# Paleogenomics/IBDGem

Hardware: AMD Instinct MI355X
Metric: SNP-sites/sec in --LD mode, chr1, 2504-indiv panel (higher is better)
Workload: dtype f64

## Files before the change

ibdgem_amd/csrc/ibdg_api.cpp:

```cpp
#include "../../include/ibdgem_hip.h"
#include "ibdg_ctx.h"
#include "ibdg_kernels.h"
#include "ibdg_states.h"

static_assert(sizeof(ibdg_segment) == 56, "ibdg_segment has no padding");

#include <hip/hip_runtime.h>

#include <cerrno>
#include <unistd.h>
#include <cfloat>
#include <cmath>
#include <cstdarg>
#include <cstdio>
#include <cstdlib>
#include <cstring>
#include <algorithm>
#include <atomic>
#include <chrono>
#include <mutex>
#include <string>
#include <thread>
#include <vector>

// ... 1333 lines not shown
}

int relayout_when_paid(ibdg_ctx *c, size_t T)
{
    if (!(c->tab.pop_lut_ok && c->lay.pop_sites_ok && !c->lay.compact && c->opt.compact == 0 && c->opt.variant != 1 &&
          c->opt.variant != 3 && c->lay.pop_dense_enough))
        return 0;
    const bool to_mfma = c->opt.mfma_targets && c->lay.tab_in_lds && T >= (size_t)c->opt.mfma_min;
    c->lay.relayout_credit += to_mfma ? (uint64_t)((T + IBDG_TG - 1) / IBDG_TG) * 20u : (uint64_t)T * (c->opt.mx_counts ? 12u : 16u);
    if (c->lay.relayout_credit >= (uint64_t)std::max<long>(1, c->opt.compact_targets)) {
        if (quiesce(c)) return 1;
        Built b = build_segments(c, true);
        if (b == Built::not_applicable)
            b = build_segments(c, false);
        return b == Built::failed;
    }
    return 0;
}

struct RunPlan {
    size_t T = 0, lanes = 0;
    bool ld = false, use_pop = false;
    int variant = 0, count_unit = 0;
    bool recount = false, rows_on_main = false, dispatch_events = false, rt_build = false;
    size_t MT = 0, n_gg = 0, T_g = 0, gg_batch = 0, T_cnt = 0, n_grp = 0, T_one = 0;
    bool mfma_wg_sum = false;
    size_t ph_group = 0, part_bytes = 0;
    int mx_counts = 0;
    long rho_shift = 0;
    bool ibd1 = false, ibd0_pass = false, fin_in_next = false, end_in_dispatch = false;
    bool side_fast = false;
    unsigned row_blocks = 0;
};

int plan_run(ibdg_ctx *c, size_t T, size_t lanes, int ld_mode, bool row_table, RunPlan &P)
{
    P.T = T; P.lanes = lanes; P.ld = ld_mode != 0;
    P.rt_build = row_table && !c->rt.fresh(*c);
    if (ld_mode) {
        const bool can = c->tab.pop_lut_ok && c->lay.pop_sites_ok && (c->lay.compact ? c->lay.t32c.p : c->pan.t32.p);
        if (c->opt.variant == 2 && !can)
            return fail(c, "[::] ERROR in ibdg_run: ld_variant 2 (exponent counting) is not applicable here "
                           "(clamped P(D|G) table, epsilon outside (0,1), max_cov > 50 or rows out of order)");
        P.use_pop = can && c->opt.variant != 1 && c->opt.variant != 3 && (c->opt.variant == 2 || c->lay.pop_dense_enough);
    }
    P.variant = ld_mode ? (P.use_pop ? 2 : (c->opt.variant == 3 ? 3 : 1)) : 0;
    P.recount = c->opt.count_in_run || !c->pan.counts_valid;
    P.rows_on_main = !ld_mode && !P.recount;
    P.dispatch_events = P.use_pop && c->opt.dispatch_events && c->sites.n_win > 0;
    if (P.use_pop) {
        P.MT = (size_t)ibdg::ld_popcount_mt_width();
        const bool mt_fits = ibdg::ld_popcount_lds_bytes(c->lay.max_seg, c->lay.wpg, c->lay.ct_max + 1, c->lay.tab_in_lds, c->lay.seg_ring,
                                                         1) <= 150 * 1024;
// ... 8 lines not shown
        }
        P.T_cnt = T - P.T_g;
        P.n_grp = (c->opt.multi_target && mt_fits && P.T_cnt >= P.MT) ? P.T_cnt / P.MT : 0;
        P.T_one = P.T_cnt - P.n_grp * P.MT;
        const size_t mem_cap = std::max<size_t>((size_t)1 << 30, c->dev_mem_bytes / 16);
        const size_t fit = std::min(c->lay.n_segs ? mem_cap / ((size_t)c->lay.n_segs * 1024) : P.n_gg, mem_cap / P.ph_group);
        P.gg_batch = std::min({std::max<size_t>(fit, 1), (size_t)std::max<long>(1, c->opt.mfma_batch), P.n_gg});
        const double log2_rho = std::log2(c->tab.eps / (1 - c->tab.eps)), log2_sigma = std::log2(0.5 / (1 - c->tab.eps));
        const bool shift8 = (double)(c->lay.ct_max + 1) * std::max(std::fabs(log2_rho + 8.0), std::fabs(log2_sigma)) <= 1000.0;
        P.rho_shift = shift8 ? 8 : std::lround(-log2_rho);
        const double per_read = std::max(std::fabs(log2_rho + (double)P.rho_shift), std::fabs(log2_sigma));
        P.mx_counts = c->opt.mx_counts && P.rho_shift >= 0 && P.rho_shift <= 40 &&
                      (!c->lay.tab_in_lds || (double)(c->lay.ct_max + 1) * per_read <= 1000.0) &&
                      ibdg::ld_popcount_lds_bytes(c->lay.max_seg, c->lay.wpg, c->lay.ct_max + 1, c->lay.tab_in_lds, c->lay.seg_ring, 2) <= 150 * 1024;
        P.part_bytes = T * (size_t)c->sites.n_win * c->pan.n_chunks * 16;
        const bool p2_stale = !c->p2.fresh(*c, P.mx_counts);
        if (P.T_one && P.mx_counts && c->lay.tab_in_lds && c->opt.ibd0_after > 0) {
            if (!c->ibd0.fresh(*c))
                c->ibd0.made(*c);
            c->ibd0.ibd0_runs += P.T_one;
            P.ibd1 = !p2_stale || (P.n_gg > 0) || c->ibd0.ibd0_runs >= (uint64_t)c->opt.ibd0_after;
        }
        P.ibd0_pass = p2_stale && (P.n_gg > 0 || P.ibd1);
        P.fin_in_next = c->opt.fin_next && c->opt.async && P.T_one > 0 && P.T_one == P.T_cnt && P.n_gg == 0;
        P.end_in_dispatch = c->opt.end_in_dispatch && P.fin_in_next && !P.dispatch_events && P.T_one == T && !c->opt.log_windows;
        P.count_unit = P.T_one ? (P.mx_counts ? (P.ibd1 ? 3 : 2) : 1) : 0;
        P.side_fast = P.n_gg > 0;
    }
    if (ld_mode && !P.recount && !P.side_fast && c->opt.site_blocks > 0)
        P.row_blocks = std::max<unsigned>(1u, (unsigned)((size_t)c->n_cu * c->opt.site_blocks / T));
    return 0;
}

int start_run(ibdg_ctx *c, const RunPlan &P, EvSet &E, bool flushed)
{
    E.recount = P.recount; E.ld = P.ld; E.rows_on_main = P.rows_on_main; E.has_kernel_times = P.dispatch_events;
    const bool chained = c->tl.chain_ok && c->opt.async;
    if (P.dispatch_events) {
        E.start = E.start_own;
        if (chained)
            HIP_TRY(c, hipStreamWaitEvent(c->stream2, c->tl.evs[c->tl.ev_head].ld_end, 0));
        return 0;
    }
    if (chained && !flushed) {
        E.start = c->tl.evs[c->tl.ev_head].ld_end;
    } else {
        HIP_TRY(c, hipEventRecord(E.start_own, c->stream));
        E.start = E.start_own;
    }
// ... 98 lines not shown
    return 0;
}

int launch_mt_groups(ibdg_ctx *c, const RunPlan &P, const ibdg::PopArgs &pa, ibdg::KernelEvents &first,
                     ibdg::KernelEvents dominant)
{
    if (ring_settle(c)) return 1;
    ibdg::PopArgs pm = pa;
    pm.mx_counts = 0;
    pm.rec_ready = (const uint32_t *)c->twords_mt.p; pm.wc_ready = (const uint32_t *)c->wtarget_mt.p;
    ibdg::launch_win_target_mt(pm, (unsigned)P.n_grp, c->stream, first);
    first = ibdg::KernelEvents();
    if (ibdg::launch_ld_popcount_mt(pm, (unsigned)P.n_grp, c->stream, P.T_one ? ibdg::KernelEvents() : dominant))
        return fail(c, "[::] ERROR in ibdg_run: the multi-target --LD kernel could not be launched");
    return 0;
}

int launch_singles(ibdg_ctx *c, const RunPlan &P, ibdg::PopArgs pa, ibdg::KernelEvents first, ibdg::KernelEvents dominant,
                   bool same_inputs, EvSet &E)
{
    Ring &R = c->ring;
    pa.t_base = (uint32_t)(P.T_g + P.n_grp * P.MT);
    pa.ibd1 = P.ibd1 ? 1u : 0u;
    const ibdg_ctx::Images::Key key = c->img.key_for(*c, pa.t_base, (uint32_t)P.T_one, P.mx_counts, (int)P.ibd1, R.cur);
    const bool wt_cached = same_inputs && c->img.fresh(key) && !P.dispatch_events;
    const bool wt_ahead = R.unsettled && !P.dispatch_events;
    const hipStream_t is = wt_ahead ? c->stream3 : c->stream;
    if (!wt_ahead && ring_settle(c)) return 1;
    if (wt_ahead && R.s3_gen != c->sites_gen) {
        HIP_TRY(c, hipEventRecord(R.ev_s3sync, c->stream));
        HIP_TRY(c, hipStreamWaitEvent(c->stream3, R.ev_s3sync, 0));
        R.s3_gen = c->sites_gen;
    }
    if (P.ibd1) {
        if (!c->fb.fresh(*c)) {
            if (ensure(c, c->fb.fragb, (size_t)c->lay.n_segs * 72)) return 1;
            if (!c->fb.ev_fb)
                HIP_TRY(c, hipEventCreateWithFlags(&c->fb.ev_fb, hipEventDisableTiming));
            ibdg::launch_frag_base(pa, (uint32_t *)c->fb.fragb.p, is);
            HIP_TRY(c, hipEventRecord(c->fb.ev_fb, is));
            HIP_TRY(c, hipStreamWaitEvent(wt_ahead ? c->stream : c->stream3, c->fb.ev_fb, 0));
            c->fb.made(*c);
        }
        pa.frag_base = (const uint32_t *)c->fb.fragb.p;
    }
    if (!wt_cached)
// ... 197 lines not shown
    const size_t lanes = (size_t)c->pan.n_groups * c->pan.cpw * 64;
    const bool want_ll = c->opt.site_results != 0;
    const bool row_table = want_ll && ld_mode;
    if (ensure(c, c->targets, Ring::SLOTS * T * 4) || (want_ll && ensure(c, c->site_ll, (row_table ? 1 : T) * c->sites.n_sites * 24)) ||
        (row_table && ensure(c, c->rt.row_tab, c->sites.n_sites * 32)) || ensure(c, c->win_ll, T * (size_t)c->sites.n_win * 24) ||
        (c->opt.log_windows && ensure(c, c->wlog.win_log2, T * (size_t)c->sites.n_win * 24)))
        return 1;
    const bool same_bg = c->bg.prev_pu == pu_id && c->bg.prev_has_bg == (bg_count ? 1 : 0) && c->bg.prev_lanes == lanes &&
                         (!bg_count || (c->bg.prev_bg.size() == c->pan.n_ids &&
                                        std::equal(bg_count, bg_count + c->pan.n_ids, c->bg.prev_bg.begin()))) &&
                         c->bg.base_w.p;
    const bool same_inputs = same_bg && c->prev_targets.size() == T && std::equal(targets, targets + T, c->prev_targets.begin()) &&
                             c->weight.p;
    if (!same_bg && set_background(c, bg_count, pu_id, lanes)) return 1;
    if (ring_settle(c) || (!same_inputs && ring_prepare(c, targets, T, lanes))) return 1;
    if (ld_mode && relayout_when_paid(c, T)) return 1;
    RunPlan P;
    if (plan_run(c, T, lanes, ld_mode, row_table, P)) return 1;
    const bool ld_log = c->opt.log_windows && ld_mode && c->sites.n_win > 0;
    if (ld_log && ld_log_refused(c))
        return fail(c, "[::] ERROR in ibdg_run: log_windows cannot give the --LD columns here: %s", ld_log_refused(c));
    c->last_variant = P.variant;
    c->last_count_unit = P.count_unit;
    const bool flush = c->fin.pending && (!same_bg || c->fin.sites_gen != c->sites_gen || !P.use_pop || P.ibd0_pass ||
                                          !P.fin_in_next || c->fin.count != (unsigned)P.T_cnt || c->fin.args.t_base != (uint32_t)P.T_g);
    if (flush && flush_finalize(c)) return 1;
    const int ev_slot = (c->tl.ev_head + 1) % ibdg_ctx::Timeline::EV_RING;
    EvSet &E = c->tl.evs[ev_slot];
    if (start_run(c, P, E, flush)) return 1;

    const ibdg::RowsArgs sa = rows_args(c, ld_mode, row_table);
    if (ld_log && launch_log_windows(c, P)) return 1;
    if (P.use_pop ? launch_pop(c, P, E, same_inputs) : ld_mode && launch_strict(c, P, targets, bg_count, pu_id)) return 1;
    if (ring_settle(c)) return 1;
    if (P.rows_on_main) {
        if (join_streams(c)) return 1;
        unsigned blocks = 0;
        if (c->opt.rows_blocks > 0)
            blocks = std::max<unsigned>(1u, (unsigned)((size_t)c->n_cu * c->opt.rows_blocks / T));
        ibdg::launch_rows_windows(sa, (unsigned)T, c->stream, blocks);
        if (c->opt.log_windows)
            ibdg::launch_win_log_rows(sa, (unsigned)T, (double *)c->wlog.win_log2.p, c->stream);
    }
    if (!P.dispatch_events && !P.end_in_dispatch)
        HIP_TRY(c, hipEventRecord(E.ld_end, c->stream));
    if (!P.rows_on_main && queue_stream2(c, P, sa, E)) return 1;
// ... 400 lines not shown
    if (back + 1 >= (unsigned)ibdg_ctx::Timeline::EV_RING || (long)back >= c->tl.runs_done)
        return fail(c, "[::] ERROR in ibdg_run_kernel_ms: no timing kept for the run %u calls back", back);
    const EvSet &E = c->tl.evs[(c->tl.ev_head + ibdg_ctx::Timeline::EV_RING - (int)back) % ibdg_ctx::Timeline::EV_RING];
    if (!E.has_kernel_times)
        return fail(c, "[::] ERROR in ibdg_run_kernel_ms: that run did not use the exponent-counting --LD kernel");
    if (quiesce(c)) return 1;
    HIP_TRY(c, hipEventElapsedTime(ms, E.k_start, E.k_stop));
    return 0;
}

int ibdg_last_run_ms(ibdg_ctx *c, float out[5])
{
    if (!c || !out) return 1;
    if (c->tl.runs_done == 0) {
        for (int i = 0; i < 5; ++i) out[i] = 0.f;
        return 0;
    }
    return ibdg_run_ms(c, 0, out);
}

int ibdg_last_ld_variant(const ibdg_ctx *c) { return c ? c->last_variant : 0; }

int ibdg_last_count_unit(const ibdg_ctx *c) { return c ? c->last_count_unit : 0; }

int ibdg_ld_layout(const ibdg_ctx *c)
{
    if (!c || !c->sites.sites_valid || !c->lay.pop_sites_ok)
        return 0;
    return c->lay.compact ? 2 : 1;
}

int ibdg_set_option(ibdg_ctx *c, const char *name, long value)
{
    if (!c || !name) return 1;
    for (const OptionRow &o : OPTION_TABLE) {
        if (strcmp(name, o.name))
            continue;
        const bool in_set = o.kind == OptionRow::SET && value >= 0 && value < 63 && ((o.lo >> value) & 1);
        if ((o.kind == OptionRow::RANGE && (value < o.lo || value > o.hi)) || (o.kind == OptionRow::SET && !in_set)) {
            if (o.text)
                return fail(c, "[::] ERROR in ibdg_set_option: %s must be %s", o.name, o.text);
            return fail(c, "[::] ERROR in ibdg_set_option: %s must be %ld..%ld", o.name, o.lo, o.hi);
        }
        if (o.effect == OptionRow::JOIN_STREAMS && join_streams(c)) return 1;
        if (o.effect == OptionRow::FIX_WPG) c->opt.wpg_fixed = true;
        c->opt.*o.member = o.kind == OptionRow::BOOL ? value != 0 : o.kind == OptionRow::CLAMP ? std::min(std::max(value, o.lo), o.hi) : value;
// ... 44 lines not shown
```

ibdgem_amd/csrc/ibdg_ctx.h:

```cpp
#pragma once
#include "ibdg_kernels.h"

#include <hip/hip_runtime.h>

#include <climits>
#include <cstddef>
#include <cstdint>
#include <initializer_list>
#include <string>
#include <vector>

struct DevBuf {
    void *p = nullptr;
    size_t cap = 0;
    uint64_t allocs = 0;
    void release()
    {
        if (p)
            (void)hipFree(p);
        p = nullptr;
        cap = 0;
    }
};

// ... 28 lines not shown
        long cpw = 0;
        long waves = 8;
        long variant = 0;
        std::vector<uint32_t> bg_order;
        long wpg = 16;
        bool wpg_fixed = false;
        long multi_target = 1;
        long mfma_targets = 1;
        long mfma_plain_tau = 1;
        long mfma_min = 4;
        long mfma_wg_sum = 1;
        long mfma_batch = 36;
        long guided = 4;
        long ring = 2;
        long recbytes = 12 * 1024;
        long site_blocks = 2;
        long recount_blocks = 4;
        long compact = 0;
        long ibd0_after = 8;
        long prep_ahead = 1;
        long end_in_dispatch = 1;
        long fin_next = 1;
        long sum_dpp = 1;
        long mx_counts = 1;
        long reserve_compact = 1;
        long compact_align = 1;
        long compact_density = 4;
        long compact_targets = 256;
        long site_results = 1;
        long staged_upload = 1;
        long log_windows = 0;
        long stage_workers = Staging::WORKERS;
    } opt;

    struct Tables {
        double eps = 0.02;
        unsigned max_cov = 20;
        std::vector<double> lut_h;
        DevBuf lut;
        bool pop_lut_ok = false;
        std::vector<unsigned long> nck_h;
        DevBuf nck_dev;
        std::vector<ibdg::PowEntry> p1_h, p2_h, p3_h;
        std::vector<ibdg::WinRaw> pb_h;
        DevBuf pow1, pow2, pow3, powb;
        size_t tab_dev = 0;
// ... 167 lines not shown
        bool fresh(Product k, const int64_t want[3]) const
        { return have[k] && P[k][0] == want[0] && P[k][1] == want[1] && P[k][2] == want[2]; }
        void made(Product k, const int64_t made_for[3])
        { have[k] = true; P[k][0] = made_for[0]; P[k][1] = made_for[1]; P[k][2] = made_for[2]; }
        bool records_fresh() const { return recs_ok; }
        void records_made() { recs_ok = true; }
        void records_drop() { recs_ok = false; }
        void drop() { have[PATH] = have[POST] = recs_ok = false; }
        void free_bufs() { release_all({&path, &score, &count, &post, &pout, &ptab, &spos, &sout, &soff, &recs}); }
    } ls;

    struct PendingFin {
        bool pending = false;
        ibdg::PopFinalArgs args;
        unsigned count = 0;
        uint64_t sites_gen = 0;
        int half = 0;
    } fin;

    DevBuf wtarget_mt, twords_mt, partial, aimg, wc_slot, partial_h, vals, order;

    int last_variant = 0;
    int last_count_unit = 0;
    std::vector<uint32_t> prev_targets;
    struct Ring {
        static constexpr int SLOTS = 4;
        static constexpr int NREF_SLOTS = 2 * SLOTS;
        static constexpr size_t AHEAD_MAX_T = 64;
        static constexpr int STAGE_SLOTS = 4;
        uint32_t *stage[STAGE_SLOTS] = {};
        size_t stage_cap = 0;
        hipEvent_t stage_ev[STAGE_SLOTS] = {};
        int stage_next = 0;
        int cur = 0;
        int nref = 0;
        hipEvent_t main_read[SLOTS] = {}, s2_read[SLOTS] = {};
        bool main_pending[SLOTS] = {}, s2_pending[SLOTS] = {};
        hipEvent_t ready = nullptr;
        bool unsettled = false;
        hipEvent_t ev_s3sync = nullptr;
        uint64_t s3_gen = 0;
    } ring;

    DevBuf targets, weight, nrefpanel, af, site_ll, win_ll;
    DevBuf llr_seg, llr_part, llr_out;
    size_t n_targets = 0;
// ... 30 lines not shown
using Opt = ibdg_ctx::Options;
const OptionRow OPTION_TABLE[] = {
    {"count_in_run", &Opt::count_in_run, OptionRow::BOOL},
    {"multi_target", &Opt::multi_target, OptionRow::BOOL},
    {"mfma_targets", &Opt::mfma_targets, OptionRow::BOOL},
    {"mfma_plain_tau", &Opt::mfma_plain_tau, OptionRow::BOOL},
    {"mfma_min", &Opt::mfma_min, OptionRow::RANGE, 1, IBDG_TG},
    {"guided_runs", &Opt::guided, OptionRow::ANY},
    {"compact_align", &Opt::compact_align, OptionRow::SET, opt_set({1, 2, 4, 8, 16, 32}), 0, "1, 2, 4, 8, 16 or 32"},
    {"mfma_wg_sum", &Opt::mfma_wg_sum, OptionRow::BOOL},
    {"mfma_batch_groups", &Opt::mfma_batch, OptionRow::CLAMP, 1, 64},
    {"ibd0_after", &Opt::ibd0_after, OptionRow::CLAMP, 0, LONG_MAX},
    {"end_in_dispatch", &Opt::end_in_dispatch, OptionRow::BOOL},
    {"prep_ahead", &Opt::prep_ahead, OptionRow::BOOL},
    {"dispatch_events", &Opt::dispatch_events, OptionRow::BOOL},
    {"async", &Opt::async, OptionRow::BOOL},
    {"dev_inputs_ready", &Opt::dev_inputs_ready, OptionRow::BOOL},
    {"staged_upload", &Opt::staged_upload, OptionRow::BOOL},
    {"stage_workers", &Opt::stage_workers, OptionRow::RANGE, 1, ibdg_ctx::Staging::WORKERS},
    {"compact_tiles", &Opt::compact, OptionRow::RANGE, -1, 1, "-1 (never), 0 (auto) or 1 (always)"},
    {"finalize_in_next", &Opt::fin_next, OptionRow::RANGE, 0, 1, "0 or 1", OptionRow::JOIN_STREAMS},
    {"sum_dpp", &Opt::sum_dpp, OptionRow::RANGE, 0, 1, "0 or 1"},
    {"mx_counts", &Opt::mx_counts, OptionRow::RANGE, 0, 1, "0 or 1"},
    {"reserve_compact", &Opt::reserve_compact, OptionRow::RANGE, 0, 1, "0 or 1"},
    {"compact_density", &Opt::compact_density, OptionRow::RANGE, 1, 1000000},
    {"compact_targets", &Opt::compact_targets, OptionRow::RANGE, 1, 65536},
    {"site_results", &Opt::site_results, OptionRow::RANGE, 0, 1, "0 or 1"},
    {"log_windows", &Opt::log_windows, OptionRow::RANGE, 0, 1, "0 or 1"},
    {"rows_blocks_per_cu", &Opt::rows_blocks, OptionRow::RANGE, 0, 128},
    {"site_blocks_per_cu", &Opt::site_blocks, OptionRow::RANGE, 0, 128},
    {"recount_blocks_per_cu", &Opt::recount_blocks, OptionRow::RANGE, 0, 128},
    {"chunks_per_wave", &Opt::cpw, OptionRow::RANGE, 0, 5},
    {"waves_per_block", &Opt::waves, OptionRow::RANGE, 1, 8},
    {"ld_variant", &Opt::variant, OptionRow::RANGE, 0, 3, "0 (auto), 1 (strict), 2 (exponent counting) or 3 (reference order)"},
    {"ring_slots", &Opt::ring, OptionRow::SET, opt_set({2, 3, 4, 8}), 0, "2, 3, 4 or 8"},
    {"record_lds_bytes", &Opt::recbytes, OptionRow::RANGE, 1024, 96 * 1024},
    {"windows_per_wave", &Opt::wpg, OptionRow::RANGE, 1, 65536, nullptr, OptionRow::FIX_WPG},
};
```

ibdgem_amd/csrc/ibdg_kernels.h:

```cpp
#pragma once
#include <hip/hip_runtime_api.h>
#include <hip/hip_vector_types.h>
#include <stddef.h>
#include <stdint.h>

struct ibdg_segment;

namespace ibdg {

struct RowsArgs {
    const uint64_t *panel;
    uint32_t stride;
    uint32_t n_ids;
    const uint2 *rec_all;
    size_t n_sites;
    const double *lut;
    const uint32_t *alt_count;
    const double *pow_tab;
    const double *fo;
    const uint32_t *targets;
    const uint4 *t32;
    uint32_t n_pairs;
    const uint32_t *cov_site;
    const uint2 *rec_cov;
// ... 72 lines not shown
    const uint32_t *run_begin;
    uint32_t n_runs;
    uint32_t n_cgroups;
    uint32_t waves_per_group;
    const uint32_t *wc_ready;
    const PowEntry *pow_1me;
    const PowEntry *pow_eps;
    const uint32_t *targets;
    uint32_t t_base;
    const double *weight;
    uint32_t lanes;
    double *partial;
    uint32_t ring_slots;
    uint32_t tab_len;
    uint32_t tab_in_lds;
    uint32_t rho_shift = 0;
    const double *fin_prev = nullptr;
    const int *n_refpanel = nullptr;
    double *win_ll = nullptr;
    uint32_t sum_dpp = 0;
    uint32_t mx_counts = 0;
    double *p2_out = nullptr;
    uint32_t ibd1 = 0;
    const double *fin_p2c = nullptr, *fin_p2w = nullptr;
    const uint32_t *fin_targets = nullptr;
    const uint32_t *frag_base = nullptr;
};

struct KernelEvents {
    hipEvent_t start = nullptr, stop = nullptr;
};

struct PopFinalArgs {
    const WinConst *wconst;
    const double *partial;
    uint32_t n_win, n_chunks;
    const int *n_refpanel;
    double *win_ll;
    uint32_t t_base = 0;
    uint32_t halves = 0;
    uint32_t p_t0 = 0;
    const double *p2c = nullptr, *p2w = nullptr;
    const uint32_t *targets = nullptr;
    uint32_t lanes = 0;
};

// ... 183 lines not shown
```

ibdgem_amd/csrc/ibdg_ld_popcount.hip:

```cpp
#include "ibdg_kernels.h"
#include "ibdg_ld_dev.h"
#include "ibdg_ld_layout.h"

#include <hip/hip_runtime.h>
#include <hip/hip_ext.h>

#include <type_traits>

#ifndef IBDG_TILE_AUX
#define IBDG_TILE_AUX 2
#endif

namespace ibdg {

typedef int mx_v8i __attribute__((ext_vector_type(8)));
typedef float mx_v4f __attribute__((ext_vector_type(4)));
typedef uint32_t mx_u4 __attribute__((ext_vector_type(4)));
typedef uint32_t mx_u2 __attribute__((ext_vector_type(2)));


__device__ __forceinline__ mx_v8i bits_to_fp4(uint32_t x)
{
    mx_v8i b = {0, 0, 0, 0, 0, 0, 0, 0};
    b[0] = (int)(x & 0x11111111u);
// ... 53 lines not shown
    v = swz_add<2>(v);
    v = swz_add<4>(v);
    v = swz_add<8>(v);
    v = swz_add<16>(v);
    return v;
}

__device__ __forceinline__ double wave_sum2_dpp(double a, double b, uint32_t scr_w, uint32_t scr_r)
{
    uint4 r;
    asm volatile("ds_write_b64 %1, %2\n\t"
                 "ds_write_b64 %1, %3 offset:512\n\t"
                 "ds_read_b128 %0, %4\n\t"
                 "s_waitcnt lgkmcnt(0)"
                 : "=&v"(r)
                 : "v"(scr_w), "v"(a), "v"(b), "v"(scr_r)
                 : "memory");
    double v = __hiloint2double((int)r.y, (int)r.x) + __hiloint2double((int)r.w, (int)r.z);
    v = dpp_add<0xB1, 0xf>(v);
    v = dpp_add<0x4E, 0xf>(v);
    v = dpp_add<0x141, 0xf>(v);
    v = dpp_add<0x140, 0xf>(v);
    v = dpp_add<0x142, 0xa>(v);
    return v;
}



__device__ __forceinline__ void lds_fetch(uint4 &h0, uint4 &h1, uint2 &x, uint32_t rec_addr, uint32_t x_addr)
{
    asm volatile("ds_read_b128 %0, %3\n\t"
                 "ds_read_b128 %1, %3 offset:16\n\t"
                 "ds_read_b64 %2, %4\n\t"
                 "s_waitcnt lgkmcnt(0)"
                 : "=&v"(h0), "=&v"(h1), "=&v"(x)
                 : "v"(rec_addr), "v"(x_addr)
                 : "memory");
}

#define IBDG_PAIR_SET(tmp, a, b, cnt) \
    "v_and_b32 %[" #tmp "], %[" #a "], %[" #b "]\n\ts_nop 0\n\tv_bcnt_u32_b32 %[" #cnt "], %[" #tmp "], 0\n\t"
#define IBDG_PAIR_ADD(tmp, a, b, cnt) \
    "v_and_b32 %[" #tmp "], %[" #a "], %[" #b "]\n\ts_nop 0\n\tv_bcnt_u32_b32 %[" #cnt "], %[" #tmp "], %[" #cnt "]\n\t"
#define IBDG_COV_PLANE_TEXT(P, k) \
    P(u0, x0, cov##k, c0##k) P(u1, x1, cov##k, c1##k) P(t, hom, cov##k, ch##k) \
    P(t, u0, at0, g00##k) P(t, u1, at0, g01##k) P(t, u0, at1, g10##k) P(t, u1, at1, g11##k)
// ... 634 lines not shown
            window_end_entries<false>(r, a, t, w, wgt, k0, k1, u, m32);
    }
    ring.drain();
}

__device__ __forceinline__ double ibd1_window_value(const Run &r, const PopArgs &a, const MxCounts &m, uint32_t w, double wgt)
{
    uint4 k0, k1;
    read_window_constants(k0, k1, r, w);
    const int eK = (int)k0.x;
    const uint32_t kc0 = k0.z, kc1 = k0.w, kb0 = k1.x, kb1 = k1.y;
    uint32_t ad[8];
    ad[0] = mad24<8>(__float_as_uint(m.acc0[2]), kb0);   ad[1] = mad24<8>(__float_as_uint(m.acc0[0]), kc0);
    ad[2] = mad24<8>(__float_as_uint(m.acc1[2]), kb0);   ad[3] = mad24<8>(__float_as_uint(m.acc1[0]), kc0);
    ad[4] = mad24<8>(__float_as_uint(m.acc0[3]), kb1);   ad[5] = mad24<8>(__float_as_uint(m.acc0[1]), kc1);
    ad[6] = mad24<8>(__float_as_uint(m.acc1[3]), kb1);   ad[7] = mad24<8>(__float_as_uint(m.acc1[1]), kc1);
    uint2 pq[8];
    lds_read_pow8_b64(pq, ad);
    double val[4];
    ld_products_plain<4>(pq, ad, eK, r.tab1, a.rho_shift, val);
    return wgt * (((val[0] + val[1]) + val[2]) + val[3]);
}

template <class Ring>
__device__ __forceinline__ void run_ibd1_form(Ring &ring, const Run &r, const PopArgs &a, unsigned t)
{
    const double wgt = a.weight[(size_t)(a.t_base + t) * a.lanes + r.c * 64 + r.lane];
    ring.wait_first();
    MxCounts m = {{0.f, 0.f, 0.f, 0.f}, {0.f, 0.f, 0.f, 0.f}, {0, 0, 0, 0}, {0, 0}};
    mx_v4f bias4 = {12582912.f, 12582912.f, 12582912.f, 12582912.f};
    asm volatile("" : "+v"(bias4));
    SegCursor cur = {0, r.rec_addr + 24 * (r.lane & 3), r.x_off0, 0};
    uint32_t w = r.w0;
    while (cur.s < r.nseg) {
        uint32_t flags = segment_x1<true>(ring, cur, r, m, bias4);
        while (!(flags & (1u << 15)))
            flags = segment_x1<false>(ring, cur, r, m, bias4);
        const double tot = wave_sum_lane63_only(ibd1_window_value(r, a, m, w, wgt));
        if (r.lane == 63)
            partial_of(a, r, t, w)[1] = tot;
        ++w;
    }
    ring.drain();
}

__device__ __forceinline__ bool fused_finalize(uint32_t &bx, unsigned t, const WinConst *__restrict__ wconst, const PopArgs &a)
{
    if (!a.fin_prev)
        return false;
    const uint32_t n_fin = (a.n_win + a.waves_per_group - 1) / a.waves_per_group;
    if (bx >= n_fin) {
        bx -= n_fin;
        return false;
    }
    const unsigned wave = __builtin_amdgcn_readfirstlane(threadIdx.x >> 6), lane = threadIdx.x & 63;
    const uint32_t w = bx * a.waves_per_group + wave;
    if (w < a.n_win) {
        const unsigned tt = a.t_base + t;
        double t0 = 0.0, t1 = 0.0;
        chunk_partial_sums(reinterpret_cast<const double2 *>(a.fin_prev) + ((size_t)tt * a.n_win + w) * a.n_chunks, a.n_chunks, lane,
                           t0, t1);
        finalize_window(t0, t1, a.fin_p2c, a.fin_p2w, a.fin_targets, a.lanes, a.n_chunks, a.n_win, w, tt, lane, wconst,
                        a.n_refpanel, a.win_ll, "fused finalize");
    }
    return true;
}

template <int NS, bool TAB_LDS, bool MX, bool IBD1 = false>
__global__ __launch_bounds__(512) void k_ld_popcount(const uint4 *__restrict__ t32,
                                                     const Seg *__restrict__ segs,
                                                     const uint32_t *__restrict__ rec_ready,
                                                     const WinConst *__restrict__ wconst,
                                                     const uint32_t *__restrict__ wc_ready,
                                                     const uint4 *__restrict__ pow_1me,
                                                     const uint4 *__restrict__ pow_eps,
                                                     const uint32_t *__restrict__ run_begin,
                                                     PopArgs a)
{
    static_assert(!IBD1 || (MX && TAB_LDS), "the IBD1 form exists with the counts on the matrix cores and the tables in LDS");
    extern __shared__ __attribute__((aligned(16))) char smem[];
    const unsigned t = blockIdx.z;
    uint32_t bx = blockIdx.x;
    if (fused_finalize(bx, t, wconst, a))
        return;
    const RunSpan sp = run_span(bx, run_begin, wconst, a);
    if (sp.nseg == 0)
        return;
    TileRing<NS, MX> ring;
    const Run r = run_prologue<MX ? IBDG_RECX_WORDS : IBDG_REC_WORDS, IBDG_WC_WORDS, TAB_LDS, MX && TAB_LDS ? 8 : 16, !IBD1>(
        sp, ring, smem, t, t32, segs, rec_ready, wc_ready, pow_1me, pow_eps, a);
    if (!r.has_chunk)
        return;
    if constexpr (IBD1)
        run_ibd1_form(ring, r, a, t);
    else if constexpr (MX)
        run_matrix_form<TAB_LDS>(ring, r, a, t);
    else
        run_vector_form<TAB_LDS>(ring, r, a, t);
}


template <int NS, bool TAB_LDS>
__global__ __launch_bounds__(512) void k_ld_popcount_mt(const uint4 *__restrict__ t32,
                                                        const Seg *__restrict__ segs,
                                                        const uint32_t *__restrict__ rec_ready,
                                                        const WinConst *__restrict__ wconst,
                                                        const uint32_t *__restrict__ wc_ready,
                                                        const uint4 *__restrict__ pow_1me,
                                                        const uint4 *__restrict__ pow_eps,
                                                        const uint32_t *__restrict__ run_begin,
                                                        PopArgs a)
{
    constexpr int TB = IBDG_MT;
    extern __shared__ __attribute__((aligned(16))) char smem[];
    const unsigned g = blockIdx.z;
    const RunSpan sp = run_span(blockIdx.x, run_begin, wconst, a);
    if (sp.nseg == 0)
// ... 71 lines not shown
    if (w >= a.n_win)
        return;
    const unsigned lane = threadIdx.x & 63;
    const unsigned t = blockIdx.y + a.t_base;
    double t0 = 0.0, t1 = 0.0;
    if (a.halves) {
        const double2 *p = reinterpret_cast<const double2 *>(a.partial) + ((size_t)(t - a.p_t0) * a.n_win + w) * a.n_chunks * 2;
        for (uint32_t c = lane; c < a.n_chunks; c += 64) {
            const double2 v = p[2 * c], u = p[2 * c + 1];
            t0 += v.x + u.x;
            t1 += v.y + u.y;
        }
    } else {
        chunk_partial_sums(reinterpret_cast<const double2 *>(a.partial) + ((size_t)(t - a.p_t0) * a.n_win + w) * a.n_chunks,
                           a.n_chunks, lane, t0, t1);
    }
    finalize_window(t0, t1, a.p2c, a.p2w, a.targets, a.lanes, a.n_chunks, a.n_win, w, t, lane, a.wconst, a.n_refpanel, a.win_ll,
                    "k_ld_finalize");
}

size_t ld_popcount_lds_bytes(uint32_t max_seg, uint32_t win_per_group, uint32_t tab_len, int tab_in_lds,
                             int ring_slots, int multi_target)
{
    const bool mt = multi_target == 1, mx = multi_target == 2 || multi_target == 3;
    return ld_lds_layout(max_seg, win_per_group, tab_len, mt ? IBDG_RECM_WORDS : mx ? IBDG_RECX_WORDS : IBDG_REC_WORDS,
                         mt ? IBDG_WCM_WORDS : IBDG_WC_WORDS, tab_in_lds ? (mx ? 8 : 16) : 0,
                         ring_slots, 8, multi_target != 3)
        .bytes;
}

template <class F>
static int with_ring_slots(uint32_t ring_slots, F &&launch)
{
    switch (ring_slots) {
    case 2:
        return launch(std::integral_constant<int, 2>());
    case 3:
        return launch(std::integral_constant<int, 3>());
    case 4:
        return launch(std::integral_constant<int, 4>());
    default:
        return launch(std::integral_constant<int, 8>());
    }
}

using CountKernel = void (*)(const uint4 *, const Seg *, const uint32_t *, const WinConst *, const uint32_t *, const uint4 *,
                             const uint4 *, const uint32_t *, PopArgs);
static int launch_counting(CountKernel kern, size_t lds, const PopArgs &a, dim3 grid, hipStream_t st, KernelEvents ev)
{
    if (hipFuncSetAttribute(reinterpret_cast<const void *>(kern), hipFuncAttributeMaxDynamicSharedMemorySize,
                            (int)lds) != hipSuccess)
        return 1;
    hipExtLaunchKernelGGL(kern, grid, dim3(64 * a.waves_per_group), (uint32_t)lds, st, ev.start, ev.stop, 0,
                          (const uint4 *)a.t32, a.segs, a.rec_ready, a.wconst, a.wc_ready, (const uint4 *)a.pow_1me,
                          (const uint4 *)a.pow_eps, a.run_begin, a);
    return 0;
}

template <int NS, bool TAB, bool MX, bool IBD1 = false>
static int launch_pop(const PopArgs &a, dim3 grid, hipStream_t st, KernelEvents ev)
{
    return launch_counting(k_ld_popcount<NS, TAB, MX, IBD1>,
                           ld_popcount_lds_bytes(a.max_seg, a.win_per_group, a.tab_len, TAB, NS, IBD1 ? 3 : MX ? 2 : 0), a, grid,
                           st, ev);
}

int launch_ld_popcount(const PopArgs &a, unsigned n_targets, int planes, hipStream_t st, KernelEvents ev)
{
    if (a.n_win == 0)
        return 0;
    if (planes < 1 || planes > 8)
        return 1;
    dim3 grid(a.n_runs * a.n_cgroups + (a.fin_prev ? (a.n_win + a.waves_per_group - 1) / a.waves_per_group : 0), 1, n_targets);
    if (a.ibd1 && (!a.mx_counts || !a.tab_in_lds || a.p2_out))
        return 1;
    return with_ring_slots(a.ring_slots, [&](auto ns) {
        constexpr int NS = decltype(ns)::value;
        if (a.ibd1)
            return launch_pop<NS, true, true, true>(a, grid, st, ev);
        if (a.mx_counts)
            return a.tab_in_lds ? launch_pop<NS, true, true>(a, grid, st, ev) : launch_pop<NS, false, true>(a, grid, st, ev);
        return a.tab_in_lds ? launch_pop<NS, true, false>(a, grid, st, ev) : launch_pop<NS, false, false>(a, grid, st, ev);
    });
}

int launch_ld_popcount_mt(const PopArgs &a, unsigned n_groups, hipStream_t st, KernelEvents ev)
{
    if (a.n_win == 0 || n_groups == 0)
        return 0;
    dim3 grid(a.n_runs * a.n_cgroups, 1, n_groups);
    return with_ring_slots(a.ring_slots, [&](auto ns) {
        constexpr int NS = decltype(ns)::value;
        const size_t lds = ld_popcount_lds_bytes(a.max_seg, a.win_per_group, a.tab_len, a.tab_in_lds != 0, NS, 1);
        return launch_counting(a.tab_in_lds ? k_ld_popcount_mt<NS, true> : k_ld_popcount_mt<NS, false>, lds, a, grid, st, ev);
    });
}

void launch_ld_finalize(const PopFinalArgs &a, unsigned n_targets, hipStream_t st, KernelEvents ev)
{
    if (a.n_win == 0)
        return;
    hipExtLaunchKernelGGL(k_ld_finalize, dim3((a.n_win + 3) / 4, n_targets), dim3(256), 0, st, ev.start, ev.stop, 0, a);
// ... 4 lines not shown
```

ibdgem_amd/engine.py:

```python
import ctypes as C
import os

import numpy as np

LIB_PATH = os.environ.get("IBDG_LIB") or os.path.join(os.path.dirname(os.path.abspath(__file__)), "libibdgem_hip.so")

_P = C.c_void_p
SYMBOLS = {
    "ibdg_abi_version": (C.c_int, []),
    "ibdg_device_count": (C.c_int, []),
    "ibdg_create": (_P, [C.c_int, C.c_double, C.c_uint]),
    "ibdg_destroy": (None, [_P]),
    "ibdg_last_error": (C.c_char_p, [_P]),
    "ibdg_pdg_table": (C.c_int, [C.c_double, C.c_uint, _P]),
    "ibdg_pdg_ibd0": (C.c_double, [C.c_double] * 4),
    "ibdg_pdg_ibd1": (C.c_double, [C.c_uint, C.c_uint] + [C.c_double] * 4),
    "ibdg_row_words": (C.c_size_t, [C.c_uint]),
    "ibdg_pack_alleles": (None, [_P, C.c_uint, _P]),
    "ibdg_pack_hap_text": (C.c_int, [C.c_char_p, C.c_uint, _P]),
    "ibdg_upload_panel": (C.c_int, [_P, _P, C.c_size_t, C.c_uint]),
    "ibdg_upload_panel_dev": (C.c_int, [_P, _P, C.c_size_t, C.c_uint]),
    "ibdg_upload_sites": (C.c_int, [_P, _P, _P, _P, _P, C.c_size_t, C.c_uint]),
    "ibdg_upload_sites_dev": (C.c_int, [_P, _P, _P, _P, _P, C.c_size_t, C.c_uint]),
    "ibdg_upload_candidates": (C.c_int, [_P, _P, _P, _P, _P, C.c_size_t]),
# ... 12 lines not shown
    "ibdg_get_site_af": (C.c_int, [_P, _P]),
    "ibdg_get_site_ll": (C.c_int, [_P, C.c_size_t, _P]),
    "ibdg_get_window_ll": (C.c_int, [_P, C.c_size_t, _P]),
    "ibdg_get_window_ll_all": (C.c_int, [_P, _P]),
    "ibdg_get_window_log2": (C.c_int, [_P, C.c_size_t, _P]),
    "ibdg_get_window_log2_all": (C.c_int, [_P, _P]),
    "ibdg_window_llr_sums": (C.c_int, [_P, _P, _P, C.c_size_t, _P]),
    "ibdg_window_log2_llr_sums": (C.c_int, [_P, _P, _P, C.c_size_t, _P]),
    "ibdg_log2_states_host": (C.c_int, [_P, C.c_size_t, C.c_double, C.c_double, C.c_double, _P, _P, _P]),
    "ibdg_window_log2_states": (C.c_int, [_P, C.c_double, C.c_double, C.c_double, _P, _P, _P]),
    "ibdg_log2_posteriors_host": (C.c_int, [_P, C.c_size_t, C.c_double, C.c_double, C.c_double, _P, _P, _P]),
    "ibdg_window_log2_posteriors": (C.c_int, [_P, C.c_double, C.c_double, C.c_double, _P, _P, _P]),
    "ibdg_log2_segments_host": (C.c_int, [_P, C.c_size_t, C.c_double, C.c_double, C.c_double, C.c_int, _P, _P, _P, C.c_size_t,
                                          _P, _P]),
    "ibdg_window_log2_segments": (C.c_int, [_P, C.c_double, C.c_double, C.c_double, C.c_int, _P, _P, _P, _P]),
    "ibdg_get_log2_segments": (C.c_int, [_P, _P, C.c_size_t]),
    "ibdg_get_alt_counts": (C.c_int, [_P, C.c_size_t, C.c_size_t, _P]),
    "ibdg_last_run_ms": (C.c_int, [_P, _P]),
    "ibdg_run_ms": (C.c_int, [_P, C.c_uint, _P]),
    "ibdg_run_kernel_ms": (C.c_int, [_P, C.c_uint, _P]),
    "ibdg_last_ld_variant": (C.c_int, [_P]),
    "ibdg_ld_layout": (C.c_int, [_P]),
    "ibdg_last_count_unit": (C.c_int, [_P]),
    "ibdg_set_option": (C.c_int, [_P, C.c_char_p, C.c_long]),
    "ibdg_set_background_order": (C.c_int, [_P, _P, C.c_size_t]),
    "ibdg_selftest": (C.c_int, [C.c_char_p]),
    "ibdg_sync": (C.c_int, [_P]),
}


class EngineError(RuntimeError):
    pass


_lib = None


def load_library(path=LIB_PATH):
    global _lib
    if _lib is not None and path == LIB_PATH:
        return _lib
    if not os.path.exists(path):
        raise EngineError(f"{path} not found: build it with `make -C ibdgem_amd/csrc` "
                          "(python -c 'import __graft_entry__ as g; g.build()'). There is no CPU fallback.")
    lib = C.CDLL(path)
    for name, (res, args) in SYMBOLS.items():
# ... 343 lines not shown
        self._chk(self.lib.ibdg_last_run_ms(self.ctx, out))
        return dict(total=out[0], alt_count=out[1], rows=out[2], ld=out[3])

    def run_ms(self, back):
        out = (C.c_float * 5)()
        self._chk(self.lib.ibdg_run_ms(self.ctx, back, out))
        return dict(total=out[0], alt_count=out[1], rows=out[2], ld=out[3])

    def run_kernel_ms(self, back=0):
        out = C.c_float()
        self._chk(self.lib.ibdg_run_kernel_ms(self.ctx, back, C.byref(out)))
        return out.value

    def set_background_order(self, ids):
        a = np.ascontiguousarray([] if ids is None else ids, dtype=np.uint32)
        self._chk(self.lib.ibdg_set_background_order(self.ctx, a.ctypes.data if len(a) else None, len(a)))

    def last_ld_variant(self):
        return self.lib.ibdg_last_ld_variant(self.ctx)

    def last_count_unit(self):
        return self.lib.ibdg_last_count_unit(self.ctx)

    def ld_layout(self):
        return self.lib.ibdg_ld_layout(self.ctx)

    def sync(self):
        self._chk(self.lib.ibdg_sync(self.ctx))
```

include/ibdgem_hip.h:

```cpp
#ifndef IBDGEM_HIP_H
#define IBDGEM_HIP_H

#include <stddef.h>
#include <stdint.h>

#ifdef __cplusplus
extern "C" {
#endif

#define IBDG_ABI_VERSION 5

typedef struct ibdg_ctx ibdg_ctx;

int ibdg_abi_version(void);

int ibdg_device_count(void);

ibdg_ctx *ibdg_create(int device, double epsilon, unsigned max_cov);

void ibdg_destroy(ibdg_ctx *ctx);

const char *ibdg_last_error(const ibdg_ctx *ctx);

int ibdg_pdg_table(double epsilon, unsigned max_cov, double *out);
// ... 71 lines not shown
    double post_min;
} ibdg_segment;
int ibdg_log2_segments_host(const double *log2_tab, size_t n_win, double p01, double p02, double p12, int with_post,
                            const uint64_t *pos_first, const uint64_t *pos_last, ibdg_segment *seg, size_t seg_cap,
                            uint64_t *n_seg, uint64_t summary[12]);
int ibdg_window_log2_segments(ibdg_ctx *ctx, double p01, double p02, double p12, int with_post, const uint64_t *pos_first,
                              const uint64_t *pos_last, uint64_t *n_seg, uint64_t *summary);
int ibdg_get_log2_segments(ibdg_ctx *ctx, ibdg_segment *seg, size_t cap);
int ibdg_get_alt_counts(ibdg_ctx *ctx, size_t first_row, size_t n, uint32_t *out);


int ibdg_last_run_ms(ibdg_ctx *ctx, float out[5]);

int ibdg_run_ms(ibdg_ctx *ctx, unsigned back, float out[5]);

int ibdg_run_kernel_ms(ibdg_ctx *ctx, unsigned back, float *ms);

int ibdg_last_ld_variant(const ibdg_ctx *ctx);

int ibdg_ld_layout(const ibdg_ctx *ctx);

int ibdg_last_count_unit(const ibdg_ctx *ctx);

int ibdg_set_option(ibdg_ctx *ctx, const char *name, long value);

int ibdg_set_background_order(ibdg_ctx *ctx, const uint32_t *ids, size_t n);

int ibdg_selftest(const char *what);

int ibdg_sync(ibdg_ctx *ctx);

#ifdef __cplusplus
}
#endif
#endif
```

Measured before the change: 7.147 billion.

## Pair consecutive IBD1 window reductions into one LDS-staged DPP wave sum

```diff
diff --git a/ibdgem_amd/csrc/ibdg_api.cpp b/ibdgem_amd/csrc/ibdg_api.cpp
--- a/ibdgem_amd/csrc/ibdg_api.cpp
+++ b/ibdgem_amd/csrc/ibdg_api.cpp
@@ -1379,6 +1379,7 @@
     size_t T = 0, lanes = 0;
     bool ld = false, use_pop = false;
     int variant = 0, count_unit = 0;
+    int window_end = 0;
     bool recount = false, rows_on_main = false, dispatch_events = false, rt_build = false;
     size_t MT = 0, n_gg = 0, T_g = 0, gg_batch = 0, T_cnt = 0, n_grp = 0, T_one = 0;
     bool mfma_wg_sum = false;
@@ -1386,6 +1387,7 @@
     int mx_counts = 0;
     long rho_shift = 0;
     bool ibd1 = false, ibd0_pass = false, fin_in_next = false, end_in_dispatch = false;
+    bool pair_sums = false;
     bool side_fast = false;
     unsigned row_blocks = 0;
 };
@@ -1440,9 +1442,17 @@
             P.ibd1 = !p2_stale || (P.n_gg > 0) || c->ibd0.ibd0_runs >= (uint64_t)c->opt.ibd0_after;
         }
         P.ibd0_pass = p2_stale && (P.n_gg > 0 || P.ibd1);
+        if (P.ibd1 && c->opt.pair_sums) {
+            const auto per_cu = [&](int form) {
+                return std::min<size_t>(4, (size_t)160 * 1024 / ibdg::ld_popcount_lds_bytes(c->lay.max_seg, c->lay.wpg, c->lay.ct_max + 1,
+                                                                                           c->lay.tab_in_lds, c->lay.seg_ring, form));
+            };
+            P.pair_sums = per_cu(4) == per_cu(3);
+        }
         P.fin_in_next = c->opt.fin_next && c->opt.async && P.T_one > 0 && P.T_one == P.T_cnt && P.n_gg == 0;
         P.end_in_dispatch = c->opt.end_in_dispatch && P.fin_in_next && !P.dispatch_events && P.T_one == T && !c->opt.log_windows;
         P.count_unit = P.T_one ? (P.mx_counts ? (P.ibd1 ? 3 : 2) : 1) : 0;
+        P.window_end = P.T_one ? (P.pair_sums ? 2 : 1) : 0;
         P.side_fast = P.n_gg > 0;
     }
     if (ld_mode && !P.recount && !P.side_fast && c->opt.site_blocks > 0)
@@ -1587,6 +1597,7 @@
     Ring &R = c->ring;
     pa.t_base = (uint32_t)(P.T_g + P.n_grp * P.MT);
     pa.ibd1 = P.ibd1 ? 1u : 0u;
+    pa.pair_sums = P.pair_sums ? 1u : 0u;
     const ibdg_ctx::Images::Key key = c->img.key_for(*c, pa.t_base, (uint32_t)P.T_one, P.mx_counts, (int)P.ibd1, R.cur);
     const bool wt_cached = same_inputs && c->img.fresh(key) && !P.dispatch_events;
     const bool wt_ahead = R.unsettled && !P.dispatch_events;
@@ -1830,6 +1841,7 @@
         return fail(c, "[::] ERROR in ibdg_run: log_windows cannot give the --LD columns here: %s", ld_log_refused(c));
     c->last_variant = P.variant;
     c->last_count_unit = P.count_unit;
+    c->last_window_end = P.window_end;
     const bool flush = c->fin.pending && (!same_bg || c->fin.sites_gen != c->sites_gen || !P.use_pop || P.ibd0_pass ||
                                           !P.fin_in_next || c->fin.count != (unsigned)P.T_cnt || c->fin.args.t_base != (uint32_t)P.T_g);
     if (flush && flush_finalize(c)) return 1;
@@ -2276,6 +2288,7 @@
 int ibdg_last_ld_variant(const ibdg_ctx *c) { return c ? c->last_variant : 0; }
 
 int ibdg_last_count_unit(const ibdg_ctx *c) { return c ? c->last_count_unit : 0; }
+int ibdg_last_window_end(const ibdg_ctx *c) { return c ? c->last_window_end : 0; }
 
 int ibdg_ld_layout(const ibdg_ctx *c)
 {
diff --git a/ibdgem_amd/csrc/ibdg_ctx.h b/ibdgem_amd/csrc/ibdg_ctx.h
--- a/ibdgem_amd/csrc/ibdg_ctx.h
+++ b/ibdgem_amd/csrc/ibdg_ctx.h
@@ -74,6 +74,7 @@
         long end_in_dispatch = 1;
         long fin_next = 1;
         long sum_dpp = 1;
+        long pair_sums = 1;
         long mx_counts = 1;
         long reserve_compact = 1;
         long compact_align = 1;
@@ -287,6 +288,7 @@
 
     int last_variant = 0;
     int last_count_unit = 0;
+    int last_window_end = 0;
     std::vector<uint32_t> prev_targets;
     struct Ring {
         static constexpr int SLOTS = 4;
@@ -363,6 +365,7 @@
     {"finalize_in_next", &Opt::fin_next, OptionRow::RANGE, 0, 1, "0 or 1", OptionRow::JOIN_STREAMS},
     {"sum_dpp", &Opt::sum_dpp, OptionRow::RANGE, 0, 1, "0 or 1"},
     {"mx_counts", &Opt::mx_counts, OptionRow::RANGE, 0, 1, "0 or 1"},
+    {"pair_sums", &Opt::pair_sums, OptionRow::RANGE, 0, 1, "0 or 1"},
     {"reserve_compact", &Opt::reserve_compact, OptionRow::RANGE, 0, 1, "0 or 1"},
     {"compact_density", &Opt::compact_density, OptionRow::RANGE, 1, 1000000},
     {"compact_targets", &Opt::compact_targets, OptionRow::RANGE, 1, 65536},
diff --git a/ibdgem_amd/csrc/ibdg_kernels.h b/ibdgem_amd/csrc/ibdg_kernels.h
--- a/ibdgem_amd/csrc/ibdg_kernels.h
+++ b/ibdgem_amd/csrc/ibdg_kernels.h
@@ -118,6 +118,7 @@
     uint32_t mx_counts = 0;
     double *p2_out = nullptr;
     uint32_t ibd1 = 0;
+    uint32_t pair_sums = 0;
     const double *fin_p2c = nullptr, *fin_p2w = nullptr;
     const uint32_t *fin_targets = nullptr;
     const uint32_t *frag_base = nullptr;
diff --git a/ibdgem_amd/csrc/ibdg_ld_popcount.hip b/ibdgem_amd/csrc/ibdg_ld_popcount.hip
--- a/ibdgem_amd/csrc/ibdg_ld_popcount.hip
+++ b/ibdgem_amd/csrc/ibdg_ld_popcount.hip
@@ -99,6 +99,29 @@
     v = dpp_add<0x141, 0xf>(v);
     v = dpp_add<0x140, 0xf>(v);
     v = dpp_add<0x142, 0xa>(v);
+    return v;
+}
+
+__device__ __forceinline__ void wave_sum_park(double a, uint32_t scr_w)
+{
+    asm volatile("ds_write_b64 %0, %1" : : "v"(scr_w), "v"(a) : "memory");
+}
+
+__device__ __forceinline__ double wave_sum_pair_dpp(double b, uint32_t scr_w, uint32_t scr_r)
+{
+    uint4 r;
+    asm volatile("ds_write_b64 %1, %2 offset:512\n\t"
+                 "ds_read_b128 %0, %3\n\t"
+                 "s_waitcnt lgkmcnt(0)"
+                 : "=&v"(r)
+                 : "v"(scr_w), "v"(b), "v"(scr_r)
+                 : "memory");
+    double v = __hiloint2double((int)r.y, (int)r.x) + __hiloint2double((int)r.w, (int)r.z);
+    v = dpp_add<0xB1, 0xf>(v);
+    v = dpp_add<0x4E, 0xf>(v);
+    v = dpp_add<0x141, 0xf>(v);
+    v = dpp_add<0x140, 0xf>(v);
+    v = dpp_add<0x142, 0xf>(v);
     return v;
 }
 
@@ -779,7 +802,7 @@
     return wgt * (((val[0] + val[1]) + val[2]) + val[3]);
 }
 
-template <class Ring>
+template <bool PAIR, class Ring>
 __device__ __forceinline__ void run_ibd1_form(Ring &ring, const Run &r, const PopArgs &a, unsigned t)
 {
     const double wgt = a.weight[(size_t)(a.t_base + t) * a.lanes + r.c * 64 + r.lane];
@@ -789,13 +812,26 @@
     asm volatile("" : "+v"(bias4));
     SegCursor cur = {0, r.rec_addr + 24 * (r.lane & 3), r.x_off0, 0};
     uint32_t w = r.w0;
-    while (cur.s < r.nseg) {
+    auto window_value = [&]() {
         uint32_t flags = segment_x1<true>(ring, cur, r, m, bias4);
         while (!(flags & (1u << 15)))
             flags = segment_x1<false>(ring, cur, r, m, bias4);
-        const double tot = wave_sum_lane63_only(ibd1_window_value(r, a, m, w, wgt));
-        if (r.lane == 63)
-            partial_of(a, r, t, w)[1] = tot;
+        return ibd1_window_value(r, a, m, w, wgt);
+    };
+    const uint32_t second = PAIR ? (r.lane >> 5) * a.n_chunks * 2 : 0;
+    while (cur.s < r.nseg) {
+        const double v = window_value();
+        if (PAIR && cur.s < r.nseg) {
+            wave_sum_park(v, r.scr_w);
+            ++w;
+            const double tot = wave_sum_pair_dpp(window_value(), r.scr_w, r.scr_r);
+            if ((r.lane & 31) == 31)
+                partial_of(a, r, t, w - 1)[1 + second] = tot;
+        } else {
+            const double tot = wave_sum_lane63_only(v);
+            if (r.lane == 63)
+                partial_of(a, r, t, w)[1] = tot;
+        }
         ++w;
     }
     ring.drain();
@@ -823,7 +859,7 @@
     return true;
 }
 
-template <int NS, bool TAB_LDS, bool MX, bool IBD1 = false>
+template <int NS, bool TAB_LDS, bool MX, bool IBD1 = false, bool PAIR = false>
 __global__ __launch_bounds__(512) void k_ld_popcount(const uint4 *__restrict__ t32,
                                                      const Seg *__restrict__ segs,
                                                      const uint32_t *__restrict__ rec_ready,
@@ -835,6 +871,7 @@
                                                      PopArgs a)
 {
     static_assert(!IBD1 || (MX && TAB_LDS), "the IBD1 form exists with the counts on the matrix cores and the tables in LDS");
+    static_assert(!PAIR || IBD1, "the paired window end is the IBD1 form's");
     extern __shared__ __attribute__((aligned(16))) char smem[];
     const unsigned t = blockIdx.z;
     uint32_t bx = blockIdx.x;
@@ -844,12 +881,12 @@
     if (sp.nseg == 0)
         return;
     TileRing<NS, MX> ring;
-    const Run r = run_prologue<MX ? IBDG_RECX_WORDS : IBDG_REC_WORDS, IBDG_WC_WORDS, TAB_LDS, MX && TAB_LDS ? 8 : 16, !IBD1>(
+    const Run r = run_prologue<MX ? IBDG_RECX_WORDS : IBDG_REC_WORDS, IBDG_WC_WORDS, TAB_LDS, MX && TAB_LDS ? 8 : 16, !IBD1 || PAIR>(
         sp, ring, smem, t, t32, segs, rec_ready, wc_ready, pow_1me, pow_eps, a);
     if (!r.has_chunk)
         return;
     if constexpr (IBD1)
-        run_ibd1_form(ring, r, a, t);
+        run_ibd1_form<PAIR>(ring, r, a, t);
     else if constexpr (MX)
         run_matrix_form<TAB_LDS>(ring, r, a, t);
     else
@@ -967,7 +1004,7 @@
 size_t ld_popcount_lds_bytes(uint32_t max_seg, uint32_t win_per_group, uint32_t tab_len, int tab_in_lds,
                              int ring_slots, int multi_target)
 {
-    const bool mt = multi_target == 1, mx = multi_target == 2 || multi_target == 3;
+    const bool mt = multi_target == 1, mx = multi_target >= 2 && multi_target <= 4;
     return ld_lds_layout(max_seg, win_per_group, tab_len, mt ? IBDG_RECM_WORDS : mx ? IBDG_RECX_WORDS : IBDG_REC_WORDS,
                          mt ? IBDG_WCM_WORDS : IBDG_WC_WORDS, tab_in_lds ? (mx ? 8 : 16) : 0,
                          ring_slots, 8, multi_target != 3)
@@ -1002,12 +1039,12 @@
     return 0;
 }
 
-template <int NS, bool TAB, bool MX, bool IBD1 = false>
+template <int NS, bool TAB, bool MX, bool IBD1 = false, bool PAIR = false>
 static int launch_pop(const PopArgs &a, dim3 grid, hipStream_t st, KernelEvents ev)
 {
-    return launch_counting(k_ld_popcount<NS, TAB, MX, IBD1>,
-                           ld_popcount_lds_bytes(a.max_seg, a.win_per_group, a.tab_len, TAB, NS, IBD1 ? 3 : MX ? 2 : 0), a, grid,
-                           st, ev);
+    return launch_counting(k_ld_popcount<NS, TAB, MX, IBD1, PAIR>,
+                           ld_popcount_lds_bytes(a.max_seg, a.win_per_group, a.tab_len, TAB, NS, IBD1 ? (PAIR ? 4 : 3) : MX ? 2 : 0), a,
+                           grid, st, ev);
 }
 
 int launch_ld_popcount(const PopArgs &a, unsigned n_targets, int planes, hipStream_t st, KernelEvents ev)
@@ -1019,10 +1056,12 @@
     dim3 grid(a.n_runs * a.n_cgroups + (a.fin_prev ? (a.n_win + a.waves_per_group - 1) / a.waves_per_group : 0), 1, n_targets);
     if (a.ibd1 && (!a.mx_counts || !a.tab_in_lds || a.p2_out))
         return 1;
+    if (a.pair_sums && !a.ibd1)
+        return 1;
     return with_ring_slots(a.ring_slots, [&](auto ns) {
         constexpr int NS = decltype(ns)::value;
         if (a.ibd1)
-            return launch_pop<NS, true, true, true>(a, grid, st, ev);
+            return a.pair_sums ? launch_pop<NS, true, true, true, true>(a, grid, st, ev) : launch_pop<NS, true, true, true>(a, grid, st, ev);
         if (a.mx_counts)
             return a.tab_in_lds ? launch_pop<NS, true, true>(a, grid, st, ev) : launch_pop<NS, false, true>(a, grid, st, ev);
         return a.tab_in_lds ? launch_pop<NS, true, false>(a, grid, st, ev) : launch_pop<NS, false, false>(a, grid, st, ev);
diff --git a/ibdgem_amd/engine.py b/ibdgem_amd/engine.py
--- a/ibdgem_amd/engine.py
+++ b/ibdgem_amd/engine.py
@@ -58,6 +58,7 @@
     "ibdg_last_ld_variant": (C.c_int, [_P]),
     "ibdg_ld_layout": (C.c_int, [_P]),
     "ibdg_last_count_unit": (C.c_int, [_P]),
+    "ibdg_last_window_end": (C.c_int, [_P]),
     "ibdg_set_option": (C.c_int, [_P, C.c_char_p, C.c_long]),
     "ibdg_set_background_order": (C.c_int, [_P, _P, C.c_size_t]),
     "ibdg_selftest": (C.c_int, [C.c_char_p]),
@@ -447,6 +448,9 @@
     def last_count_unit(self):
         return self.lib.ibdg_last_count_unit(self.ctx)
 
+    def last_window_end(self):
+        return self.lib.ibdg_last_window_end(self.ctx)
+
     def ld_layout(self):
         return self.lib.ibdg_ld_layout(self.ctx)
 
diff --git a/include/ibdgem_hip.h b/include/ibdgem_hip.h
--- a/include/ibdgem_hip.h
+++ b/include/ibdgem_hip.h
@@ -117,6 +117,8 @@
 
 int ibdg_last_count_unit(const ibdg_ctx *ctx);
 
+int ibdg_last_window_end(const ibdg_ctx *ctx);
+
 int ibdg_set_option(ibdg_ctx *ctx, const char *name, long value);
 
 int ibdg_set_background_order(ibdg_ctx *ctx, const uint32_t *ids, size_t n);
```

New measurement: 7.359 billion (median of 6 runs). 3.0% higher.
